# vovw/algonauts-2025

Hardware: AMD Instinct MI355X
Metric: TRs/sec trimodal encode to 1000 parcels (higher is better)
Workload: dtype bf16; 1 GPU; trimodal encode, precomputed bf16 feats, per GPU B=64 sequences (4 subjects x R=16) x T=1024, L*D=4096 per modality, hidden 3072, 8 layers, V=1000 parcels, n_output_timesteps=1024; forward only; global_batch=64, seq_len=1024, parallelism=dp1

## Files before the change

### algonauts-2025_amd/csrc/gemm_common.h

```cpp
#pragma once
#include "common.h"
#include <utility>

typedef const __attribute__((address_space(1))) void* gptr_t;
typedef __attribute__((address_space(3))) void* lptr_t;

__device__ __forceinline__ float gelu_erf(float x) {
  return 0.5f * x * (1.0f + erff(x * 0.70710678118654752440f));
}

__device__ __forceinline__ int xcd_remap(int bid, int nwg) {
  const int q = nwg >> 3, r = nwg & 7, xcd = bid & 7;
  const int base = (xcd < r) ? xcd * (q + 1) : r * (q + 1) + (xcd - r) * q;
  return base + (bid >> 3);
}

__device__ __forceinline__ void tile_coords(int bid, int tiles_m, int tiles_n, int& tm, int& tn) {
#ifndef TRIBE_GEMM_BAND_ROWS
#define TRIBE_GEMM_BAND_ROWS 4
#endif
  constexpr int GM = TRIBE_GEMM_BAND_ROWS;
  const int tile = xcd_remap(bid, tiles_m * tiles_n);
  const int band = tile / (GM * tiles_n);
  const int first_m = band * GM;
  const int gm = (tiles_m - first_m < GM) ? tiles_m - first_m : GM;
  const int r = tile - band * GM * tiles_n;
  tn = r / gm;
  tm = first_m + (r - tn * gm);
}

typedef __attribute__((ext_vector_type(2))) float f32x2_t;
constexpr float GELU_POLY2_LO = -4.39382219f;
__device__ __forceinline__ f32x2_t gelu_poly2(f32x2_t v) {
  f32x2_t c;
  c.x = __builtin_amdgcn_fmed3f(v.x, GELU_POLY2_LO, 4.4f);
  c.y = __builtin_amdgcn_fmed3f(v.y, GELU_POLY2_LO, 4.4f);
  const f32x2_t t = c * c;
  f32x2_t q = 4.4347532590638394e-11f;
  q = q * t + -4.493755145773548e-09f;
  q = q * t + 2.0033526482166053e-07f;
  q = q * t + -5.224721007834887e-06f;
  q = q * t + 8.98004655027762e-05f;
  q = q * t + -0.0010902436915785074f;
  q = q * t + 0.009767354466021061f;
  q = q * t + -0.06628739088773727f;
  q = q * t + 0.3988831341266632f;
  const f32x2_t phi = c * q + 0.5f;
  return v * phi;
}

__device__ __forceinline__ float gelu_grad(float v) {
  const float cdf = 0.5f * (1.0f + erff(v * 0.70710678118654752440f));
  const float pdf = 0.3989422804014327f * __expf(-0.5f * v * v);
  return cdf + v * pdf;
}
__device__ __forceinline__ f32x2_t gelu_grad2(f32x2_t v) {
  f32x2_t c;
  c.x = __builtin_amdgcn_fmed3f(v.x, -4.4f, 4.4f);
  c.y = __builtin_amdgcn_fmed3f(v.y, -4.4f, 4.4f);
  const f32x2_t t = c * c;
  f32x2_t q = 4.4347532590638394e-11f;
  q = q * t + -4.493755145773548e-09f;
  q = q * t + 2.0033526482166053e-07f;
  q = q * t + -5.224721007834887e-06f;
  q = q * t + 8.98004655027762e-05f;
  q = q * t + -0.0010902436915785074f;
  q = q * t + 0.009767354466021061f;
  q = q * t + -0.06628739088773727f;
  q = q * t + 0.3988831341266632f;
  const f32x2_t cdf = c * q + 0.5f;
  const f32x2_t e = v * v * -0.72134752044448170368f;
  f32x2_t pdf;
  pdf.x = 0.3989422804014327f * __builtin_amdgcn_exp2f(e.x);
  pdf.y = 0.3989422804014327f * __builtin_amdgcn_exp2f(e.y);
  return cdf + v * pdf;
}
__device__ __forceinline__ void gelu_grad_mul4(float (&v)[4], const u16x4_t pre) {
  const f32x2_t lo = gelu_grad2(f32x2_t{bf16_to_f32(pre[0]), bf16_to_f32(pre[1])}), hi = gelu_grad2(f32x2_t{bf16_to_f32(pre[2]), bf16_to_f32(pre[3])});
  v[0] *= lo.x; v[1] *= lo.y; v[2] *= hi.x; v[3] *= hi.y;
}

__device__ __forceinline__ float silu_f(float v) {
  return v * __builtin_amdgcn_rcpf(1.0f + __builtin_amdgcn_exp2f(-v * 1.4426950408889634f));
}

__device__ __forceinline__ float sigmoid_f(float v) {
  return __builtin_amdgcn_rcpf(1.0f + __builtin_amdgcn_exp2f(-v * 1.4426950408889634f));
}

__device__ __forceinline__ float quad_xor1(float v) {
  return __int_as_float(__builtin_amdgcn_mov_dpp(__float_as_int(v), 0xB1, 0xF, 0xF, true));
}
__device__ __forceinline__ float quad_xor2(float v) {
  return __int_as_float(__builtin_amdgcn_mov_dpp(__float_as_int(v), 0x4E, 0xF, 0xF, true));
}

struct EpiCtx {
  const float* bias;
  const float* res;
  char* C;
  int64_t c_off;
  bool vec;
};

__device__ __forceinline__ EpiCtx make_epi_ctx(const tribe_gemm_desc& g, int64_t b1, int64_t b0, int64_t b1g) {
  EpiCtx c;
  const int64_t bb = g.gather_bias ? b1g : b1;
  c.bias = g.bias ? g.bias + bb * g.sBias1 + b0 * g.sBias0 : nullptr;
  c.res = g.res ? g.res + b1 * g.sRes1 + b0 * g.sRes0 : nullptr;
  c.C = (char*)g.C;
  c.c_off = b1 * g.sC1 + b0 * g.sC0;
  const int esz = (g.c_dtype == TRIBE_BF16) ? 2 : 4;
  bool v = ((g.ldc & 3) == 0) && ((c.c_off & 3) == 0) && ((((uintptr_t)g.C) & (uintptr_t)(4 * esz - 1)) == 0);
  if (g.bias_mode == TRIBE_BIAS_COL) v = v && ((((uintptr_t)c.bias) & 15) == 0);
  if (c.res) v = v && ((g.ldres & 3) == 0) && ((((uintptr_t)c.res) & 15) == 0);
  if (g.res_scale) v = v && ((((uintptr_t)g.res_scale) & 15) == 0);
  if (g.rowadd) v = v && ((g.ld_rowadd & 3) == 0) && ((((uintptr_t)g.rowadd) & 15) == 0);
  if (g.gadd) v = v && ((g.ld_gadd & 3) == 0) && ((((uintptr_t)g.gadd) & 15) == 0);
  if (g.aux) v = v && ((g.ld_aux & 3) == 0) && ((((uintptr_t)g.aux) & 7) == 0);
  c.vec = v;
  return c;
}

__device__ __forceinline__ void quad_transpose(f32x4_t acc, float alpha, int lane, float (&v)[4]) {
  const int a = lane & 3;
  float v0 = acc[0] * alpha, v1 = acc[1] * alpha, v2 = acc[2] * alpha, v3 = acc[3] * alpha;
  const bool b0 = a & 1, b1 = a & 2;
  const float t0 = quad_xor1(b0 ? v0 : v1), t1 = quad_xor1(b0 ? v2 : v3);
  if (b0) { v0 = t0; v2 = t1; } else { v1 = t0; v3 = t1; }
  const float u0 = quad_xor2(b1 ? v0 : v2), u1 = quad_xor2(b1 ? v1 : v3);
  if (b1) { v0 = u0; v1 = u1; } else { v2 = u0; v3 = u1; }
  v[0] = v0; v[1] = v1; v[2] = v2; v[3] = v3;
}

template <int OUT_BF16, int EXT>
__device__ __forceinline__ void epilogue_row4(const tribe_gemm_desc& g, const EpiCtx& c, float (&v)[4], int64_t m, int64_t n) {
  if (m >= g.M || n >= g.N) return;
  if (g.bias_mode == TRIBE_BIAS_ROW) {
    const float b = c.bias[m];
#pragma unroll
    for (int k = 0; k < 4; ++k) v[k] += b;
  }
  const float* rowadd = g.rowadd ? g.rowadd + (m % g.rowadd_period) * g.ld_rowadd : nullptr;
  const float* gadd = g.gadd ? g.gadd + g.gadd_index[m / g.gadd_div] * g.ld_gadd : nullptr;
  const int64_t idx = c.c_off + m * g.ldc + n;
  if (c.vec && n + 4 <= g.N) {
    if (g.bias_mode == TRIBE_BIAS_COL) {
      const float4 b = *(const float4*)(c.bias + n);
      v[0] += b.x; v[1] += b.y; v[2] += b.z; v[3] += b.w;
    }
    if (EXT && (g.act == TRIBE_ACT_SWIGLU || g.act == TRIBE_ACT_GLU)) {
      const bool glu = g.act == TRIBE_ACT_GLU;
      const float o0 = glu ? v[0] * sigmoid_f(v[1]) : silu_f(v[0]) * v[1];
      const float o1 = glu ? v[2] * sigmoid_f(v[3]) : silu_f(v[2]) * v[3];
      const int64_t oidx = c.c_off + m * g.ldc + (n >> 1);
      if (OUT_BF16) {
        const unsigned int pk = (unsigned int)f32_to_bf16(o0) | ((unsigned int)f32_to_bf16(o1) << 16);
        *(unsigned int*)((unsigned short*)c.C + oidx) = pk;
      } else {
        *(float2*)((float*)c.C + oidx) = make_float2(o0, o1);
      }
      return;
    }
    if (g.act == TRIBE_ACT_GELU) {
      if (EXT && g.aux) {
        u16x4_t pre;
#pragma unroll
        for (int k = 0; k < 4; ++k) pre[k] = f32_to_bf16(v[k]);
        *(u16x4_t*)((unsigned short*)g.aux + c.c_off + m * g.ld_aux + n) = pre;
      }
      if (OUT_BF16) {
        const f32x2_t lo = gelu_poly2(f32x2_t{v[0], v[1]}), hi = gelu_poly2(f32x2_t{v[2], v[3]});
        v[0] = lo.x; v[1] = lo.y; v[2] = hi.x; v[3] = hi.y;
      } else {
#pragma unroll
        for (int k = 0; k < 4; ++k) v[k] = gelu_erf(v[k]);
      }
    } else if (EXT && g.act == TRIBE_ACT_GELU_BWD) {
      const u16x4_t pre = *(const u16x4_t*)((const unsigned short*)g.aux + c.c_off + m * g.ld_aux + n);
      gelu_grad_mul4(v, pre);
    } else if (EXT && g.act == TRIBE_ACT_SILU) {
#pragma unroll
      for (int k = 0; k < 4; ++k) v[k] = silu_f(v[k]);
    } else if (EXT && g.act == TRIBE_ACT_EXP2) {
#pragma unroll
      for (int k = 0; k < 4; ++k) v[k] = __builtin_amdgcn_exp2f(v[k]);
    } else if (EXT && g.act == TRIBE_ACT_MUL_AUX) {
      const u16x4_t p = *(const u16x4_t*)((const unsigned short*)g.aux + c.c_off + m * g.ld_aux + n);
#pragma unroll
      for (int k = 0; k < 4; ++k) v[k] *= bf16_to_f32(p[k]);
    }
    if (c.res) {
      const float4 r = *(const float4*)(c.res + m * g.ldres + n);
      if (g.res_scale) {
        const float4 s = *(const float4*)(g.res_scale + n);
        v[0] += r.x * s.x; v[1] += r.y * s.y; v[2] += r.z * s.z; v[3] += r.w * s.w;
      } else {
        v[0] += r.x; v[1] += r.y; v[2] += r.z; v[3] += r.w;
      }
    }
    if (rowadd) {
      const float4 r = *(const float4*)(rowadd + n);
      v[0] += r.x; v[1] += r.y; v[2] += r.z; v[3] += r.w;
    }
    if (gadd) {
      const float4 r = *(const float4*)(gadd + n);
      v[0] += r.x; v[1] += r.y; v[2] += r.z; v[3] += r.w;
    }
    if (OUT_BF16) {
      u16x4_t o;
#pragma unroll
      for (int k = 0; k < 4; ++k) o[k] = f32_to_bf16(v[k]);
      *(u16x4_t*)((unsigned short*)c.C + idx) = o;
    } else {
      *(float4*)((float*)c.C + idx) = make_float4(v[0], v[1], v[2], v[3]);
    }
    return;
  }
  if (EXT && (g.act == TRIBE_ACT_SWIGLU || g.act == TRIBE_ACT_GLU)) {
#pragma unroll
    for (int k = 0; k < 4; k += 2) {
      if (n + k + 1 >= g.N) break;
      float gate = v[k], up = v[k + 1];
      if (g.bias_mode == TRIBE_BIAS_COL) { gate += c.bias[n + k]; up += c.bias[n + k + 1]; }
      const float o = (g.act == TRIBE_ACT_GLU) ? gate * sigmoid_f(up) : silu_f(gate) * up;
      const int64_t oidx = c.c_off + m * g.ldc + ((n + k) >> 1);
      if (OUT_BF16) ((unsigned short*)c.C)[oidx] = f32_to_bf16(o);
      else ((float*)c.C)[oidx] = o;
    }
    return;
  }
#pragma unroll
  for (int k = 0; k < 4; ++k) {
    if (n + k >= g.N) break;
    float x = v[k];
    if (g.bias_mode == TRIBE_BIAS_COL) x += c.bias[n + k];
    if (g.act == TRIBE_ACT_GELU) {
      if (EXT && g.aux) ((unsigned short*)g.aux)[c.c_off + m * g.ld_aux + n + k] = f32_to_bf16(x);
      x = OUT_BF16 ? gelu_poly2(f32x2_t{x, x}).x : gelu_erf(x);
    } else if (EXT && g.act == TRIBE_ACT_GELU_BWD) {
      x *= gelu_grad(bf16_to_f32(((const unsigned short*)g.aux)[c.c_off + m * g.ld_aux + n + k]));
    } else if (EXT && g.act == TRIBE_ACT_SILU) x = silu_f(x);
    else if (EXT && g.act == TRIBE_ACT_EXP2) x = __builtin_amdgcn_exp2f(x);
    else if (EXT && g.act == TRIBE_ACT_MUL_AUX) x *= bf16_to_f32(((const unsigned short*)g.aux)[c.c_off + m * g.ld_aux + n + k]);
    if (c.res) {
      const float r = c.res[m * g.ldres + n + k];
      x += g.res_scale ? r * g.res_scale[n + k] : r;
    }
    if (rowadd) x += rowadd[n + k];
    if (gadd) x += gadd[n + k];
    if (OUT_BF16) ((unsigned short*)c.C)[idx + k] = f32_to_bf16(x);
    else ((float*)c.C)[idx + k] = x;
  }
}

template <class F, int... Is>
__device__ __forceinline__ void static_for_impl(F&& f, std::integer_sequence<int, Is...>) {
  (f(std::integral_constant<int, Is>{}), ...);
}
template <int N, class F>
__device__ __forceinline__ void static_for(F&& f) {
  static_for_impl(f, std::make_integer_sequence<int, N>{});
}

template <int OUT_BF16, int NI, int NJ, int EXT, int TACC = 0>
__device__ __forceinline__ void epilogue_fast(const tribe_gemm_desc& g, const EpiCtx& c, f32x4_t (&acc)[NI][NJ], int64_t mw, int64_t nw, int lane,
                                              char* lds_wave) {
  constexpr int RI = NI >= 4 ? 4 : NI;
  static_assert(NI % RI == 0 && NJ >= 1 && NJ <= 4, "accumulator grid");
  const int tq = lane >> 4;
  const int64_t row0 = TACC ? mw + (lane & 15) : mw + ((lane >> 4) << 2) + (lane & 3);
  const int64_t col0 = TACC ? nw + 4 * ((tq & 1) * 2 + (tq >> 1)) : nw + (((lane & 15) >> 2) << 2);
  const int64_t colp = nw + 16 * (lane >> 5) + 8 * (tq & 1);
  const bool bias_col = g.bias_mode == TRIBE_BIAS_COL, bias_row = g.bias_mode == TRIBE_BIAS_ROW;
  const bool res_scaled = c.res && g.res_scale;
  const bool pair_act = EXT && (g.act == TRIBE_ACT_SWIGLU || g.act == TRIBE_ACT_GLU);
  float4 bcol[NJ], rsc[NJ];
  static_for<NJ>([&](auto jt) {
    constexpr int j = decltype(jt)::value;
    if (bias_col) bcol[j] = *(const float4*)(c.bias + col0 + j * 16);
    if (res_scaled) rsc[j] = *(const float4*)(g.res_scale + col0 + j * 16);
  });
  constexpr int ROUNDS = NI / RI;
  static_for<ROUNDS>([&](auto rt) {
    constexpr int round = decltype(rt)::value;
    float brow[RI], srow[RI], ssq[RI];
    static_for<RI>([&](auto it) { ssq[decltype(it)::value] = 0.f; });
    if (bias_row) {
      static_for<RI>([&](auto it) {
        const int64_t r = row0 + (round * RI + decltype(it)::value) * 16;
        brow[decltype(it)::value] = r < g.M ? c.bias[r] : 0.f;
      });
    }
    if (g.row_scale) {
      static_for<RI>([&](auto it) {
        const int64_t r = row0 + (round * RI + decltype(it)::value) * 16;
        srow[decltype(it)::value] = r < g.M ? g.row_scale[r] : 0.f;
      });
    }
    const bool tile_add = c.res || g.rowadd;
    if (tile_add) {
      static_for<RI>([&](auto it) {
        constexpr int i4 = decltype(it)::value, i = round * RI + i4;
        const int64_t r = row0 + i * 16;
        if (r < g.M) {
          const float* src = c.res ? c.res + r * g.ldres + col0
                                   : g.rowadd + (int64_t)((unsigned)r % (unsigned)g.rowadd_period) * g.ld_rowadd + col0;
          static_for<NJ>([&](auto jt) {
            constexpr int j = decltype(jt)::value;
            __builtin_amdgcn_global_load_lds((gptr_t)(src + j * 16), (lptr_t)(lds_wave + (i4 * NJ + j) * 1024), 16, 0, 0);
          });
        }
      });
      asm volatile("s_waitcnt vmcnt(0)" ::: "memory");
    }
    u16x4_t pre[EXT ? RI * NJ : 1];
    const bool gelu_bwd = EXT && g.act == TRIBE_ACT_GELU_BWD, mul_aux = EXT && g.act == TRIBE_ACT_MUL_AUX;
    if (gelu_bwd || mul_aux) {
      static_for<RI * NJ>([&](auto st) {
        constexpr int s = decltype(st)::value, i = round * RI + s / NJ, j = s % NJ;
        const int64_t r = row0 + i * 16;
        pre[EXT ? s : 0] = r < g.M ? *(const u16x4_t*)((const unsigned short*)g.aux + c.c_off + r * g.ld_aux + col0 + j * 16) : u16x4_t{0, 0, 0, 0};
      });
    }
    uint2 pend = make_uint2(0u, 0u);
    static_for<RI * NJ>([&](auto st) {
      constexpr int s = decltype(st)::value, i4 = s / NJ, i = round * RI + i4, j = s % NJ;
      const int64_t row = row0 + i * 16;
      float v[4];
      if constexpr (TACC) {
#pragma unroll
        for (int k = 0; k < 4; ++k) v[k] = acc[i][j][k] * g.alpha;
      } else {
        quad_transpose(acc[i][j], g.alpha, lane, v);
      }
      const bool live = row < g.M;
      if (!TACC && !live) return;
      if (g.row_scale) {
#pragma unroll
        for (int k = 0; k < 4; ++k) v[k] *= srow[i4];
      }
      if (bias_row) {
#pragma unroll
        for (int k = 0; k < 4; ++k) v[k] += brow[i4];
      }
      if (bias_col) { v[0] += bcol[j].x; v[1] += bcol[j].y; v[2] += bcol[j].z; v[3] += bcol[j].w; }
      if (pair_act) {
        const bool glu = g.act == TRIBE_ACT_GLU;
        const float o0 = glu ? v[0] * sigmoid_f(v[1]) : silu_f(v[0]) * v[1];
        const float o1 = glu ? v[2] * sigmoid_f(v[3]) : silu_f(v[2]) * v[3];
        const int64_t oidx = c.c_off + row * g.ldc + ((col0 + j * 16) >> 1);
        if (live) {
          if (OUT_BF16) *(unsigned int*)((unsigned short*)c.C + oidx) = (unsigned int)f32_to_bf16(o0) | ((unsigned int)f32_to_bf16(o1) << 16);
          else *(float2*)((float*)c.C + oidx) = make_float2(o0, o1);
        }
        return;
      }
      if (g.act == TRIBE_ACT_GELU) {
        if (EXT && g.aux) {
          u16x4_t p;
#pragma unroll
          for (int k = 0; k < 4; ++k) p[k] = f32_to_bf16(v[k]);
          if (live) *(u16x4_t*)((unsigned short*)g.aux + c.c_off + row * g.ld_aux + col0 + j * 16) = p;
        }
        if (OUT_BF16) {
          const f32x2_t lo = gelu_poly2(f32x2_t{v[0], v[1]}), hi = gelu_poly2(f32x2_t{v[2], v[3]});
          v[0] = lo.x; v[1] = lo.y; v[2] = hi.x; v[3] = hi.y;
        } else {
#pragma unroll
          for (int k = 0; k < 4; ++k) v[k] = gelu_erf(v[k]);
        }
      } else if (gelu_bwd) {
        gelu_grad_mul4(v, pre[EXT ? s : 0]);
      } else if (mul_aux) {
#pragma unroll
        for (int k = 0; k < 4; ++k) v[k] *= bf16_to_f32(pre[EXT ? s : 0][k]);
      } else if (EXT && g.act == TRIBE_ACT_SILU) {
#pragma unroll
        for (int k = 0; k < 4; ++k) v[k] = silu_f(v[k]);
      } else if (EXT && g.act == TRIBE_ACT_EXP2) {
#pragma unroll
        for (int k = 0; k < 4; ++k) v[k] = __builtin_amdgcn_exp2f(v[k]);
      }
      if (tile_add) {
        const float4 r = *(const float4*)(lds_wave + s * 1024 + lane * 16);
        if (res_scaled) { v[0] += r.x * rsc[j].x; v[1] += r.y * rsc[j].y; v[2] += r.z * rsc[j].z; v[3] += r.w * rsc[j].w; }
        else { v[0] += r.x; v[1] += r.y; v[2] += r.z; v[3] += r.w; }
      }
      const int64_t idx = c.c_off + row * g.ldc + col0 + j * 16;
      auto store_bf16 = [&](unsigned short* base, int64_t ld, int64_t boff) {
        u16x4_t o;
#pragma unroll
        for (int k = 0; k < 4; ++k) o[k] = f32_to_bf16(v[k]);
        constexpr bool paired = TACC && (NJ % 2 == 0 || j + 1 < NJ || (j & 1));
        if constexpr (!paired) {
          if (live) *(u16x4_t*)(base + boff + row * ld + col0 + j * 16) = o;
        } else {
          const uint2 pk = __builtin_bit_cast(uint2, o);
          if constexpr ((j & 1) == 0) {
            pend = pk;
          } else {
            const auto sx = __builtin_amdgcn_permlane32_swap(pend.x, pk.x, false, false);
            const auto sy = __builtin_amdgcn_permlane32_swap(pend.y, pk.y, false, false);
            if (live) *(uint4*)(base + boff + row * ld + colp + (j - 1) * 16) = make_uint4(sx[0], sy[0], sx[1], sy[1]);
          }
        }
      };
      if (OUT_BF16) {
        store_bf16((unsigned short*)c.C, g.ldc, c.c_off);
      } else {
        if (live) *(float4*)((float*)c.C + idx) = make_float4(v[0], v[1], v[2], v[3]);
        if (g.c_bf16) store_bf16(g.c_bf16, g.ld_c_bf16, 0);
        if (g.row_sumsq && live) ssq[i4] += v[0] * v[0] + v[1] * v[1] + v[2] * v[2] + v[3] * v[3];
      }
    });
    if (!OUT_BF16 && g.row_sumsq) {
      static_for<RI>([&](auto it) {
        constexpr int i4 = decltype(it)::value;
        float t = ssq[i4];
        t += __shfl_xor(t, TACC ? 16 : 4, 64);
        t += __shfl_xor(t, TACC ? 32 : 8, 64);
        const int64_t r = row0 + (round * RI + i4) * 16;
        if ((TACC ? lane < 16 : (lane & 12) == 0) && r < g.M) g.row_sumsq[r * g.ld_row_sumsq + (int64_t)((unsigned)nw / (unsigned)(16 * NJ))] = t;
      });
    }
  });
}

__device__ __forceinline__ float mul_unfused(float a, float b) {
#pragma clang fp contract(off)
  return a * b;
}

__device__ __forceinline__ unsigned int f32_to_plane_lo(float v) {
  const unsigned int w = __float_as_uint(v);
  return (w & 0x1ffffu) == 0x18000u ? 0x8001u : (w & 0xffffu);
}
__device__ __forceinline__ float planes_to_f32(unsigned int hi, unsigned int lo) {
  return __uint_as_float(((hi - (lo > 0x8000u ? 1u : 0u)) << 16) | lo);
}
typedef unsigned short tribe_u16x2 __attribute__((ext_vector_type(2)));
__device__ __forceinline__ void planes_to_f32x2(unsigned int hi2, unsigned int lo2, float& r0, float& r1) {
  const tribe_u16x2 a = __builtin_bit_cast(tribe_u16x2, lo2) - (tribe_u16x2)(1);
  r0 = __uint_as_float((hi2 << 16) + (unsigned int)(int)(short)a.x + 1u);
  r1 = __uint_as_float((hi2 & 0xffff0000u) + (unsigned int)(int)(short)a.y + 1u);
}
__device__ __forceinline__ unsigned int f32x2_to_plane_lo(float v0, float v1) {
  const unsigned int w0 = __float_as_uint(v0), w1 = __float_as_uint(v1);
  const unsigned int t0 = (w0 & 0x1ffffu) == 0x18000u ? 1u : 0u, t1 = (w1 & 0x1ffffu) == 0x18000u ? 1u : 0u;
  return ((w0 + t0) & 0xffffu) | ((w1 + t1) << 16);
}

__device__ __forceinline__ float sumsq4(const float (&v)[4]) {
  return ((mul_unfused(v[0], v[0]) + mul_unfused(v[1], v[1])) + mul_unfused(v[2], v[2])) + mul_unfused(v[3], v[3]);
}

template <int OUT_BF16, int ROLE, int NI, int NJ, int TACC, int PL = 0>
__device__ __forceinline__ void epilogue_role(const tribe_gemm_desc& g, f32x4_t (&acc)[NI][NJ], int64_t mw, int64_t nw, int lane, char* lds_wave) {
  constexpr bool BIAS = ROLE == TRIBE_ROLE_FF1 || ROLE == TRIBE_ROLE_FF2;
  constexpr bool GELU = ROLE == TRIBE_ROLE_FF1;
  constexpr bool RES = ROLE == TRIBE_ROLE_OUT_PROJ || ROLE == TRIBE_ROLE_FF2;
  constexpr int RI = 4, ROUNDS = NI / RI;
  static_assert(TACC == 1 && NI % RI == 0 && NJ >= 1 && NJ <= 4, "transposed accumulators, rounds of 4 sub-tile rows");
  static_assert(OUT_BF16 == (RES ? 0 : 1), "QKV / FF1 write bf16, out-proj / FF2 the f32 residual stream");
  static_assert(PL == 0 || (RES && NJ == 4 && PL >= 1 && PL <= 3), "planes: the residual roles at 256-column tiles");
  constexpr bool PL_IN = PL == 2 || PL == 3, PL_OUT = PL == 1 || PL == 2;
  const int tq = lane >> 4;
  const int64_t row0 = mw + (lane & 15);
  const int64_t col0 = nw + 4 * ((tq & 1) * 2 + (tq >> 1));
  const int64_t colp = nw + 16 * (lane >> 5) + 8 * (tq & 1);
  const int64_t left = g.M - row0;
  const int rows_left = left >= 16 * NI ? 16 * NI : (left > 0 ? (int)left : 0);
  const bool has_rs = !RES && g.row_scale != nullptr, has_rsc = RES && g.res_scale != nullptr;
  const bool has_cb = PL_OUT || (PL == 0 && RES && g.c_bf16 != nullptr), has_ssq = RES && g.row_sumsq != nullptr;
  float4 bcol[NJ], rsc[NJ];
  static_for<NJ>([&](auto jt) {
    constexpr int j = decltype(jt)::value;
    if constexpr (BIAS) bcol[j] = *(const float4*)(g.bias + col0 + j * 16);
    if constexpr (RES) rsc[j] = has_rsc ? *(const float4*)(g.res_scale + col0 + j * 16) : make_float4(1.f, 1.f, 1.f, 1.f);
  });
  unsigned short* c16 = OUT_BF16 ? (unsigned short*)g.C + row0 * g.ldc : (has_cb ? g.c_bf16 + row0 * g.ld_c_bf16 : nullptr);
  const int64_t step16 = 16 * (OUT_BF16 ? g.ldc : g.ld_c_bf16);
  float* c32 = (RES && !PL_OUT) ? (float*)g.C + row0 * g.ldc + col0 : nullptr;
  const float* rsrc = (RES && !PL_IN) ? g.res + row0 * g.ldres + col0 : nullptr;
  unsigned short* clo = PL_OUT ? (unsigned short*)g.C + row0 * g.ldc + nw : nullptr;
  const unsigned short* hsrc = PL_IN ? g.c_bf16 + row0 * g.ld_c_bf16 + nw + 8 * tq : nullptr;
  const unsigned short* lsrc = PL_IN ? (const unsigned short*)g.res + row0 * g.ldres + 2 * nw + 8 * tq : nullptr;
  const int pl_rd = (tq & 1) * 256 + (lane & 15) * 16 + (tq >> 1) * 8;
  static_for<ROUNDS>([&](auto rt) {
    constexpr int round = decltype(rt)::value;
    float srow[RI], ssq[RI];
    static_for<RI>([&](auto it) {
      constexpr int i4 = decltype(it)::value, i = round * RI + i4;
      ssq[i4] = 0.f;
      srow[i4] = (has_rs && i * 16 < rows_left) ? g.row_scale[row0 + i * 16] : 1.0f;
    });
    if constexpr (RES && !PL_IN) {
      static_for<RI>([&](auto it) {
        constexpr int i4 = decltype(it)::value, i = round * RI + i4;
        if (i * 16 < rows_left) {
          static_for<NJ>([&](auto jt) {
            constexpr int j = decltype(jt)::value;
            __builtin_amdgcn_global_load_lds((gptr_t)(rsrc + j * 16), (lptr_t)(lds_wave + (i4 * NJ + j) * 1024), 16, 0, 0);
          });
        }
        rsrc += 16 * g.ldres;
      });
      asm volatile("s_waitcnt vmcnt(0)" ::: "memory");
    }
    if constexpr (PL_IN) {
      static_for<RI>([&](auto it) {
        constexpr int i4 = decltype(it)::value, i = round * RI + i4;
        if (i * 16 < rows_left) {
          static_for<NJ / 2>([&](auto pt) {
            constexpr int jp = decltype(pt)::value;
            __builtin_amdgcn_global_load_lds((gptr_t)(hsrc + jp * 32), (lptr_t)(lds_wave + (i4 * 2 + jp) * 1024), 16, 0, 0);
            __builtin_amdgcn_global_load_lds((gptr_t)(lsrc + jp * 32), (lptr_t)(lds_wave + 8192 + (i4 * 2 + jp) * 1024), 16, 0, 0);
          });
        }
        hsrc += 16 * g.ld_c_bf16;
        lsrc += 16 * g.ldres;
      });
      asm volatile("s_waitcnt vmcnt(0)" ::: "memory");
    }
    uint2 pend = make_uint2(0u, 0u);
    uint2 pend_lo = make_uint2(0u, 0u);
    static_for<RI * NJ>([&](auto st) {
      constexpr int s = decltype(st)::value, i4 = s / NJ, i = round * RI + i4, j = s % NJ;
      const bool live = i * 16 < rows_left;
      float v[4] = {acc[i][j][0], acc[i][j][1], acc[i][j][2], acc[i][j][3]};
      if constexpr (!RES) {
#pragma unroll
        for (int k = 0; k < 4; ++k) v[k] = mul_unfused(v[k], srow[i4]);
      }
      if constexpr (BIAS) { v[0] += bcol[j].x; v[1] += bcol[j].y; v[2] += bcol[j].z; v[3] += bcol[j].w; }
      if constexpr (GELU) {
        const f32x2_t lo = gelu_poly2(f32x2_t{v[0], v[1]}), hi = gelu_poly2(f32x2_t{v[2], v[3]});
        v[0] = lo.x; v[1] = lo.y; v[2] = hi.x; v[3] = hi.y;
      }
      if constexpr (RES && !PL_IN) {
        const float4 r = *(const float4*)(lds_wave + s * 1024 + lane * 16);
        v[0] += r.x * rsc[j].x; v[1] += r.y * rsc[j].y; v[2] += r.z * rsc[j].z; v[3] += r.w * rsc[j].w;
      }
      if constexpr (PL_IN) {
        const char* slot = lds_wave + (i4 * 2 + (j >> 1)) * 1024 + (j & 1) * 512 + pl_rd;
        const uint2 h = *(const uint2*)slot, l = *(const uint2*)(slot + 8192);
        float r0, r1, r2, r3;
        planes_to_f32x2(h.x, l.x, r0, r1);
        planes_to_f32x2(h.y, l.y, r2, r3);
        v[0] = __builtin_fmaf(r0, rsc[j].x, v[0]); v[1] = __builtin_fmaf(r1, rsc[j].y, v[1]);
        v[2] = __builtin_fmaf(r2, rsc[j].z, v[2]); v[3] = __builtin_fmaf(r3, rsc[j].w, v[3]);
      }
      auto store_bf16 = [&]() {
        u16x4_t o;
#pragma unroll
        for (int k = 0; k < 4; ++k) o[k] = f32_to_bf16(v[k]);
        constexpr bool paired = NJ % 2 == 0 || j + 1 < NJ || (j & 1);
        if constexpr (!paired) {
          if (live) *(u16x4_t*)(c16 + col0 + j * 16) = o;
        } else {
          const uint2 pk = __builtin_bit_cast(uint2, o);
          if constexpr ((j & 1) == 0) {
            pend = pk;
          } else {
            const auto sx = __builtin_amdgcn_permlane32_swap(pend.x, pk.x, false, false);
            const auto sy = __builtin_amdgcn_permlane32_swap(pend.y, pk.y, false, false);
            if (live) *(uint4*)(c16 + colp + (j - 1) * 16) = make_uint4(sx[0], sy[0], sx[1], sy[1]);
          }
        }
      };
      if constexpr (OUT_BF16) {
        store_bf16();
      } else if constexpr (PL_OUT) {
        store_bf16();
        const uint2 pk = make_uint2(f32x2_to_plane_lo(v[0], v[1]), f32x2_to_plane_lo(v[2], v[3]));
        if constexpr ((j & 1) == 0) {
          pend_lo = pk;
        } else {
          const auto sx = __builtin_amdgcn_permlane32_swap(pend_lo.x, pk.x, false, false);
          const auto sy = __builtin_amdgcn_permlane32_swap(pend_lo.y, pk.y, false, false);
          if (live) *(uint4*)(clo + colp + (j - 1) * 16) = make_uint4(sx[0], sy[0], sx[1], sy[1]);
        }
        if (has_ssq && live) ssq[i4] += sumsq4(v);
      } else {
        if (live) *(float4*)(c32 + j * 16) = make_float4(v[0], v[1], v[2], v[3]);
        if (has_cb) store_bf16();
        if constexpr (PL != 0) {
          if (has_ssq && live) ssq[i4] += sumsq4(v);
        } else {
          if (has_ssq && live) ssq[i4] += v[0] * v[0] + v[1] * v[1] + v[2] * v[2] + v[3] * v[3];
        }
      }
      if constexpr (j == NJ - 1) {
        c16 += step16;
        if constexpr (RES && !PL_OUT) c32 += 16 * g.ldc;
        if constexpr (PL_OUT) clo += 16 * g.ldc;
      }
    });
    if constexpr (RES) {
      if (has_ssq) {
        static_for<RI>([&](auto it) {
          constexpr int i4 = decltype(it)::value, i = round * RI + i4;
          float t = ssq[i4];
          t += __shfl_xor(t, 16, 64);
          t += __shfl_xor(t, 32, 64);
          if (lane < 16 && i * 16 < rows_left) g.row_sumsq[(row0 + i * 16) * g.ld_row_sumsq + (int64_t)((unsigned)nw / (unsigned)(16 * NJ))] = t;
        });
      }
    }
  });
}

template <int EXT>
__device__ __forceinline__ bool epilogue_fast_ok(const tribe_gemm_desc& g, const EpiCtx& c) {
  const bool act_ok = g.act == TRIBE_ACT_NONE || g.act == TRIBE_ACT_GELU ||
                      (EXT && (g.act == TRIBE_ACT_SWIGLU || g.act == TRIBE_ACT_GLU || g.act == TRIBE_ACT_SILU || g.act == TRIBE_ACT_GELU_BWD ||
                              g.act == TRIBE_ACT_EXP2 || g.act == TRIBE_ACT_MUL_AUX));
  const bool rowadd_ok = !g.rowadd || (!c.res && g.M < (1ll << 31) && g.rowadd_period < (1ll << 31));
  return c.vec && rowadd_ok && !g.gadd && (EXT || !g.aux) && act_ok;
}

template <int OUT_BF16, int EXT, int TACC = 0>
__device__ __forceinline__ void epilogue_tile16(const tribe_gemm_desc& g, const EpiCtx& c, f32x4_t acc, int64_t mt0,
                                                int64_t nt0, int lane) {
  float v[4];
  if constexpr (TACC) {
    const int tq = lane >> 4;
#pragma unroll
    for (int k = 0; k < 4; ++k) v[k] = acc[k] * g.alpha;
    epilogue_row4<OUT_BF16, EXT>(g, c, v, mt0 + (lane & 15), nt0 + 4 * ((tq & 1) * 2 + (tq >> 1)));
  } else {
    quad_transpose(acc, g.alpha, lane, v);
    epilogue_row4<OUT_BF16, EXT>(g, c, v, mt0 + ((lane >> 4) << 2) + (lane & 3), nt0 + (((lane & 15) >> 2) << 2));
  }
}

namespace tribe_gemm_detail {
template <auto KERNEL, int THREADS, int SMEM, class... Extra>
static void launch_k(dim3 grid, hipStream_t s, const tribe_gemm_desc* d, int tiles_m, int tiles_n, const Extra&... extra) {
  raise_dynamic_lds_once<KERNEL>(SMEM);
  hipLaunchKernelGGL(KERNEL, grid, dim3(THREADS, 1, 1), SMEM, s, *d, tiles_m, tiles_n, extra...);
}
}
```

Before: 642,300 TRs/s.

## Issue both residual epilogue rounds' loads up front with a single drain

For the residual-role epilogue with two rounds and 256-column tiles, the full-tile path now issues all residual/plane loads for both rounds at once. Round 0 goes via LDS DMA (through inline asm that sets M0 directly) and round 1 goes into registers, with permlane32 swaps rearranging the plane data. This swaps the two separate vmcnt(0) drains for partial waits, so round-1 load latency overlaps round-0 compute and stores. It also adds an early waitcnt and hoists the res_scale loads. The cost is higher register pressure and fragile hand-counted vmcnt values; the old path remains for partial tiles.

```diff
diff --git a/algonauts-2025_amd/csrc/gemm_common.h b/algonauts-2025_amd/csrc/gemm_common.h
--- a/algonauts-2025_amd/csrc/gemm_common.h
+++ b/algonauts-2025_amd/csrc/gemm_common.h
@@ -455,6 +455,12 @@
   return ((mul_unfused(v[0], v[0]) + mul_unfused(v[1], v[1])) + mul_unfused(v[2], v[2])) + mul_unfused(v[3], v[3]);
 }
 
+__device__ __forceinline__ void lds_dma16_unseen(const void* gsrc, const char* lds_dst) {
+  unsigned keep;
+  asm volatile("s_mov_b32 %0, m0\n\ts_mov_b32 m0, %2\n\ts_nop 0\n\tglobal_load_lds_dwordx4 %1, off\n\ts_mov_b32 m0, %0"
+               : "=&s"(keep) : "v"(gsrc), "s"((unsigned)(uintptr_t)(lptr_t)lds_dst) : "memory");
+}
+
 template <int OUT_BF16, int ROLE, int NI, int NJ, int TACC, int PL = 0>
 __device__ __forceinline__ void epilogue_role(const tribe_gemm_desc& g, f32x4_t (&acc)[NI][NJ], int64_t mw, int64_t nw, int lane, char* lds_wave) {
   constexpr bool BIAS = ROLE == TRIBE_ROLE_FF1 || ROLE == TRIBE_ROLE_FF2;
@@ -473,12 +479,18 @@
   const int rows_left = left >= 16 * NI ? 16 * NI : (left > 0 ? (int)left : 0);
   const bool has_rs = !RES && g.row_scale != nullptr, has_rsc = RES && g.res_scale != nullptr;
   const bool has_cb = PL_OUT || (PL == 0 && RES && g.c_bf16 != nullptr), has_ssq = RES && g.row_sumsq != nullptr;
+#ifndef TRIBE_EPI_TWO_DRAINS
+  if constexpr (RES && NI / 4 == 2 && NJ == 4) __builtin_amdgcn_s_waitcnt(0x0f70);
+#endif
   float4 bcol[NJ], rsc[NJ];
   static_for<NJ>([&](auto jt) {
     constexpr int j = decltype(jt)::value;
     if constexpr (BIAS) bcol[j] = *(const float4*)(g.bias + col0 + j * 16);
-    if constexpr (RES) rsc[j] = has_rsc ? *(const float4*)(g.res_scale + col0 + j * 16) : make_float4(1.f, 1.f, 1.f, 1.f);
+    if constexpr (RES) rsc[j] = make_float4(1.f, 1.f, 1.f, 1.f);
   });
+  if constexpr (RES) {
+    if (has_rsc) static_for<NJ>([&](auto jt) { rsc[decltype(jt)::value] = *(const float4*)(g.res_scale + col0 + decltype(jt)::value * 16); });
+  }
   unsigned short* c16 = OUT_BF16 ? (unsigned short*)g.C + row0 * g.ldc : (has_cb ? g.c_bf16 + row0 * g.ld_c_bf16 : nullptr);
   const int64_t step16 = 16 * (OUT_BF16 ? g.ldc : g.ld_c_bf16);
   float* c32 = (RES && !PL_OUT) ? (float*)g.C + row0 * g.ldc + col0 : nullptr;
@@ -487,6 +499,15 @@
   const unsigned short* hsrc = PL_IN ? g.c_bf16 + row0 * g.ld_c_bf16 + nw + 8 * tq : nullptr;
   const unsigned short* lsrc = PL_IN ? (const unsigned short*)g.res + row0 * g.ldres + 2 * nw + 8 * tq : nullptr;
   const int pl_rd = (tq & 1) * 256 + (lane & 15) * 16 + (tq >> 1) * 8;
+#ifdef TRIBE_EPI_TWO_DRAINS
+  constexpr bool ONE_WAIT = false;
+#else
+  constexpr bool ONE_WAIT = RES && ROUNDS == 2 && NJ == 4;
+#endif
+  auto run = [&](auto one_t) __attribute__((always_inline)) {
+  constexpr bool ONE = decltype(one_t)::value;
+  uint4 nh[ONE && PL_IN ? RI * NJ / 2 : 1], nl[ONE && PL_IN ? RI * NJ / 2 : 1];
+  float4 nf[ONE && !PL_IN ? RI * NJ : 1];
   static_for<ROUNDS>([&](auto rt) {
     constexpr int round = decltype(rt)::value;
     float srow[RI], ssq[RI];
@@ -495,7 +516,35 @@
       ssq[i4] = 0.f;
       srow[i4] = (has_rs && i * 16 < rows_left) ? g.row_scale[row0 + i * 16] : 1.0f;
     });
-    if constexpr (RES && !PL_IN) {
+    if constexpr (RES && ONE) {
+      if constexpr (round == 0) {
+        static_for<2 * RI>([&](auto it) {
+          constexpr int i = decltype(it)::value, i4 = i % RI;
+          if constexpr (PL_IN) {
+            static_for<NJ / 2>([&](auto pt) {
+              constexpr int jp = decltype(pt)::value;
+              if constexpr (i < RI) {
+                lds_dma16_unseen(hsrc + jp * 32, lds_wave + (i4 * 2 + jp) * 1024);
+                lds_dma16_unseen(lsrc + jp * 32, lds_wave + 8192 + (i4 * 2 + jp) * 1024);
+              } else {
+                nh[ONE && PL_IN ? i4 * 2 + jp : 0] = *(const uint4*)(hsrc + jp * 32);
+                nl[ONE && PL_IN ? i4 * 2 + jp : 0] = *(const uint4*)(lsrc + jp * 32);
+              }
+            });
+            hsrc += 16 * g.ld_c_bf16;
+            lsrc += 16 * g.ldres;
+          } else {
+            static_for<NJ>([&](auto jt) {
+              constexpr int j = decltype(jt)::value;
+              if constexpr (i < RI) lds_dma16_unseen(rsrc + j * 16, lds_wave + (i4 * NJ + j) * 1024);
+              else nf[ONE && !PL_IN ? i4 * NJ + j : 0] = *(const float4*)(rsrc + j * 16);
+            });
+            rsrc += 16 * g.ldres;
+          }
+        });
+        asm volatile("s_waitcnt vmcnt(%0)" ::"n"(RI * NJ) : "memory");
+      }
+    } else if constexpr (RES && !PL_IN) {
       static_for<RI>([&](auto it) {
         constexpr int i4 = decltype(it)::value, i = round * RI + i4;
         if (i * 16 < rows_left) {
@@ -507,8 +556,7 @@
         rsrc += 16 * g.ldres;
       });
       asm volatile("s_waitcnt vmcnt(0)" ::: "memory");
-    }
-    if constexpr (PL_IN) {
+    } else if constexpr (PL_IN) {
       static_for<RI>([&](auto it) {
         constexpr int i4 = decltype(it)::value, i = round * RI + i4;
         if (i * 16 < rows_left) {
@@ -525,9 +573,10 @@
     }
     uint2 pend = make_uint2(0u, 0u);
     uint2 pend_lo = make_uint2(0u, 0u);
+    uint2 odd_h = make_uint2(0u, 0u), odd_l = make_uint2(0u, 0u);
     static_for<RI * NJ>([&](auto st) {
       constexpr int s = decltype(st)::value, i4 = s / NJ, i = round * RI + i4, j = s % NJ;
-      const bool live = i * 16 < rows_left;
+      const bool live = ONE || i * 16 < rows_left;
       float v[4] = {acc[i][j][0], acc[i][j][1], acc[i][j][2], acc[i][j][3]};
       if constexpr (!RES) {
 #pragma unroll
@@ -539,12 +588,27 @@
         v[0] = lo.x; v[1] = lo.y; v[2] = hi.x; v[3] = hi.y;
       }
       if constexpr (RES && !PL_IN) {
-        const float4 r = *(const float4*)(lds_wave + s * 1024 + lane * 16);
+        float4 r;
+        if constexpr (ONE && round == 1) r = nf[ONE && !PL_IN ? s : 0];
+        else r = *(const float4*)(lds_wave + s * 1024 + lane * 16);
         v[0] += r.x * rsc[j].x; v[1] += r.y * rsc[j].y; v[2] += r.z * rsc[j].z; v[3] += r.w * rsc[j].w;
       }
       if constexpr (PL_IN) {
-        const char* slot = lds_wave + (i4 * 2 + (j >> 1)) * 1024 + (j & 1) * 512 + pl_rd;
-        const uint2 h = *(const uint2*)slot, l = *(const uint2*)(slot + 8192);
+        uint2 h, l;
+        if constexpr (ONE && round == 1) {
+          if constexpr ((j & 1) == 0) {
+            const uint4 ph = nh[ONE && PL_IN ? s / 2 : 0], pl = nl[ONE && PL_IN ? s / 2 : 0];
+            const auto hx = __builtin_amdgcn_permlane32_swap(ph.x, ph.z, false, false), hy = __builtin_amdgcn_permlane32_swap(ph.y, ph.w, false, false);
+            const auto lx = __builtin_amdgcn_permlane32_swap(pl.x, pl.z, false, false), ly = __builtin_amdgcn_permlane32_swap(pl.y, pl.w, false, false);
+            h = make_uint2(hx[0], hy[0]); l = make_uint2(lx[0], ly[0]);
+            odd_h = make_uint2(hx[1], hy[1]); odd_l = make_uint2(lx[1], ly[1]);
+          } else {
+            h = odd_h; l = odd_l;
+          }
+        } else {
+          const char* slot = lds_wave + (i4 * 2 + (j >> 1)) * 1024 + (j & 1) * 512 + pl_rd;
+          h = *(const uint2*)slot; l = *(const uint2*)(slot + 8192);
+        }
         float r0, r1, r2, r3;
         planes_to_f32x2(h.x, l.x, r0, r1);
         planes_to_f32x2(h.y, l.y, r2, r3);
@@ -597,6 +661,10 @@
         if constexpr (PL_OUT) clo += 16 * g.ldc;
       }
     });
+    if constexpr (ONE && round == 0) {
+      if (PL == 0 && has_cb) asm volatile("s_waitcnt vmcnt(%0)" ::"n"(RI * NJ + RI * NJ / 2) : "memory");
+      else asm volatile("s_waitcnt vmcnt(%0)" ::"n"(RI * NJ) : "memory");
+    }
     if constexpr (RES) {
       if (has_ssq) {
         static_for<RI>([&](auto it) {
@@ -604,11 +672,18 @@
           float t = ssq[i4];
           t += __shfl_xor(t, 16, 64);
           t += __shfl_xor(t, 32, 64);
-          if (lane < 16 && i * 16 < rows_left) g.row_sumsq[(row0 + i * 16) * g.ld_row_sumsq + (int64_t)((unsigned)nw / (unsigned)(16 * NJ))] = t;
+          if (lane < 16 && (ONE || i * 16 < rows_left)) g.row_sumsq[(row0 + i * 16) * g.ld_row_sumsq + (int64_t)((unsigned)nw / (unsigned)(16 * NJ))] = t;
         });
       }
     }
   });
+  };
+  if constexpr (ONE_WAIT) {
+    if (g.M - mw >= 16 * NI) run(std::true_type{});
+    else run(std::false_type{});
+  } else {
+    run(std::false_type{});
+  }
 }
 
 template <int EXT>
```

Measured after the change: 642,700 TRs/s, median of 2. No clear change (+0.1%).
